# CityU-AIM-Group/SimT

Measured on AMD Instinct MI355X. Metric: training images/sec at 768x768, DeepLabv2-R101+SimT, higher is better.
Workload: dtype bf16

## Files before the change

simt_amd/csrc/bn_pool.hip:

```cpp
#include "common.h"

template <int NJ>
__device__ __forceinline__ void part_colsum8(const float* part, int nblk, int C, int c0, double* out , double (*red)[8][NJ]) {
  const int cl = threadIdx.x & 7, r = threadIdx.x >> 3;
  const int c = c0 + cl;
  double s[NJ];
#pragma unroll
  for (int j = 0; j < NJ; ++j) s[j] = 0.0;
  if (c < C) {
    int b = r;
    for (; b + 96 < nblk; b += 128) {
      float v[4][NJ];
#pragma unroll
      for (int u = 0; u < 4; ++u)
#pragma unroll
        for (int j = 0; j < NJ; ++j) v[u][j] = part[((long)(b + 32 * u) * NJ + j) * C + c];
#pragma unroll
      for (int u = 0; u < 4; ++u)
#pragma unroll
        for (int j = 0; j < NJ; ++j) s[j] += (double)v[u][j];
    }
    for (; b < nblk; b += 32)
#pragma unroll
      for (int j = 0; j < NJ; ++j) s[j] += (double)part[((long)b * NJ + j) * C + c];
// ... 35 lines not shown
    running_mean[c] = (1.f - momentum) * running_mean[c] + momentum * (float)mean;
    running_var[c] = (1.f - momentum) * running_var[c] + momentum * (float)unb;
  }
}

extern "C" int simt_bn_finalize(const float* part, int nblk, int C, long count, const float* gamma, const float* beta,
                                float* running_mean, float* running_var, float momentum, float eps, float* mean,
                                float* rstd, float* scale, float* shift, simt_stream_t stream) {
  SIMT_CHECK(part && mean && rstd && scale && shift && C > 0 && nblk > 0);
  hipLaunchKernelGGL(bn_finalize_kernel, dim3((C + 7) / 8), dim3(256), 0, (hipStream_t)stream, part, nblk, C, count,
                     gamma, beta, running_mean, running_var, momentum, eps, mean, rstd, scale, shift);
  SIMT_LAUNCH_CHECK();
  return SIMT_OK;
}

template <typename T>
__global__ void bn_apply_kernel(const T* y, const float* scale, const float* shift, const T* res, const T* y2,
                                const float* scale2, const float* shift2, T* z, unsigned char* bits, long nvec, int C, int relu) {
  const int vpr = C >> 3;
  const long i0 = (long)blockIdx.x * blockDim.x + threadIdx.x;
  const int c = (int)(i0 % vpr) << 3;
  float sc[8], sh[8], sc2[8], sh2[8];
  load8(scale + c, sc);
  load8(shift + c, sh);
  if (y2) { load8(scale2 + c, sc2); load8(shift2 + c, sh2); }
  for (long i = i0; i < nvec; i += (long)gridDim.x * blockDim.x) {
    float v[8];
    load8(y + i * 8, v);
#pragma unroll
    for (int e = 0; e < 8; ++e) v[e] = v[e] * sc[e] + sh[e];
    if (res) {
      float r[8];
      load8(res + i * 8, r);
#pragma unroll
      for (int e = 0; e < 8; ++e) v[e] += r[e];
    }
    if (y2) {
      float r[8];
      load8(y2 + i * 8, r);
#pragma unroll
      for (int e = 0; e < 8; ++e) v[e] += r[e] * sc2[e] + sh2[e];
    }
    if (relu) {
#pragma unroll
      for (int e = 0; e < 8; ++e) v[e] = v[e] > 0.f ? v[e] : 0.f;
    }
    store8(z + i * 8, v);
    if (bits) {
      unsigned b = 0;
#pragma unroll
      for (int e = 0; e < 8; ++e) b |= (v[e] > 0.f ? 1u : 0u) << e;
      bits[i] = (unsigned char)b;
    }
  }
}

static inline int ew_grid(long nvec) {
  long g = (nvec + 255) / 256;
  if (g > 256 * 16) g = 256 * 16;
  if (g < 1) g = 1;
  return (int)g;
}

extern "C" int simt_bn_apply_bits(const void* y, const float* scale, const float* shift, const void* res, const void* y2,
                                  const float* scale2, const float* shift2, void* z, unsigned char* bits, long M, int C,
                                  int relu, int dtype, simt_stream_t stream) {
  SIMT_CHECK(y && scale && shift && z && C % 8 == 0 && 256 % (C / 8) == 0);
  long nvec = M * (C / 8);
  if (dtype == SIMT_BF16)
    hipLaunchKernelGGL(bn_apply_kernel<bf16_t>, dim3(ew_grid(nvec)), dim3(256), 0, (hipStream_t)stream, (const bf16_t*)y,
                       scale, shift, (const bf16_t*)res, (const bf16_t*)y2, scale2, shift2, (bf16_t*)z, bits, nvec, C, relu);
  else
    hipLaunchKernelGGL(bn_apply_kernel<float>, dim3(ew_grid(nvec)), dim3(256), 0, (hipStream_t)stream, (const float*)y,
                       scale, shift, (const float*)res, (const float*)y2, scale2, shift2, (float*)z, bits, nvec, C, relu);
  SIMT_LAUNCH_CHECK();
  return SIMT_OK;
}
extern "C" int simt_bn_apply(const void* y, const float* scale, const float* shift, const void* res, const void* y2,
                             const float* scale2, const float* shift2, void* z, long M, int C, int relu, int dtype,
                             simt_stream_t stream) {
  return simt_bn_apply_bits(y, scale, shift, res, y2, scale2, shift2, z, nullptr, M, C, relu, dtype, stream);
}

template <typename T>
__global__ __launch_bounds__(256) void bn_bwd_reduce_kernel(const T* dz, const T* z, const T* y, const float* mean,
                                                           const float* rstd, const float* scale, const float* shift,
                                                           const T* y2, const float* mean2, const float* rstd2,
                                                           float* part, long M, int C, int rows_per_block,
                                                           int mask_mode) {
  __shared__ float red[3][256][8 + 1];
  const int vpr = C >> 3;
  const int rpar = 256 / vpr;
  const int tid = threadIdx.x;
  const int vc = tid % vpr, rl = tid / vpr;
  const int c = vc << 3;
  float mu[8], rs[8], sc[8], sh[8], mu2[8], rs2[8];
  load8(mean + c, mu);
  load8(rstd + c, rs);
  if (mask_mode == 2) { load8(scale + c, sc); load8(shift + c, sh); }
  if (y2) { load8(mean2 + c, mu2); load8(rstd2 + c, rs2); }
  float s1[8], s2[8], s3[8];
#pragma unroll
  for (int e = 0; e < 8; ++e) { s1[e] = 0.f; s2[e] = 0.f; s3[e] = 0.f; }
  long r0 = (long)blockIdx.x * rows_per_block;
  long r1 = r0 + rows_per_block;
  if (r1 > M) r1 = M;
  auto row = [&](const Raw8<T>& gq, const Raw8<T>& yq, const Raw8<T>& zq, unsigned b, const Raw8<T>& y2q) {
    float g[8], yv[8];
    raw8_unpack(gq, g);
    raw8_unpack(yq, yv);
    if (mask_mode == 1) {
      float zv[8];
      raw8_unpack(zq, zv);
#pragma unroll
      for (int e = 0; e < 8; ++e) g[e] = zv[e] > 0.f ? g[e] : 0.f;
    } else if (mask_mode == 2) {
#pragma unroll
      for (int e = 0; e < 8; ++e) g[e] = (yv[e] * sc[e] + sh[e]) > 0.f ? g[e] : 0.f;
    } else if (mask_mode == 3) {
#pragma unroll
      for (int e = 0; e < 8; ++e) g[e] = ((b >> e) & 1u) ? g[e] : 0.f;
    }
#pragma unroll
    for (int e = 0; e < 8; ++e) {
      s1[e] += g[e];
      s2[e] += g[e] * ((yv[e] - mu[e]) * rs[e]);
    }
    if (y2) {
      float y2v[8];
      raw8_unpack(y2q, y2v);
#pragma unroll
      for (int e = 0; e < 8; ++e) s3[e] += g[e] * ((y2v[e] - mu2[e]) * rs2[e]);
    }
  };
  if (rl < rpar) {
    constexpr int UR = 4;
    long r = r0 + rl;
    for (; r + (long)(UR - 1) * rpar < r1; r += (long)UR * rpar) {
      Raw8<T> gq[UR], yq[UR], zq[UR], y2q[UR];
      unsigned b[UR];
#pragma unroll
      for (int u = 0; u < UR; ++u) {
        const long off = (r + (long)u * rpar) * C + c;
        raw8_load(dz + off, gq[u]);
        raw8_load(y + off, yq[u]);
        if (mask_mode == 1) raw8_load(z + off, zq[u]); else zq[u] = gq[u];
        b[u] = mask_mode == 3 ? ((const unsigned char*)z)[off >> 3] : 0u;
        if (y2) raw8_load(y2 + off, y2q[u]); else y2q[u] = gq[u];
      }
#pragma unroll
      for (int u = 0; u < UR; ++u) row(gq[u], yq[u], zq[u], b[u], y2q[u]);
    }
    for (; r < r1; r += rpar) {
      const long off = r * C + c;
      Raw8<T> gq, yq, zq, y2q;
      raw8_load(dz + off, gq);
      raw8_load(y + off, yq);
      if (mask_mode == 1) raw8_load(z + off, zq); else zq = gq;
      const unsigned b = mask_mode == 3 ? ((const unsigned char*)z)[off >> 3] : 0u;
      if (y2) raw8_load(y2 + off, y2q); else y2q = gq;
      row(gq, yq, zq, b, y2q);
    }
  }
#pragma unroll
  for (int e = 0; e < 8; ++e) { red[0][tid][e] = s1[e]; red[1][tid][e] = s2[e]; red[2][tid][e] = s3[e]; }
  __syncthreads();
  for (int idx = tid; idx < 3 * C; idx += 256) {
    int j = idx / C, cc = idx - j * C;
    int v = cc >> 3, e = cc & 7;
    float s = 0.f;
    for (int q = 0; q < rpar; ++q) s += red[j][q * vpr + v][e];
    part[((long)blockIdx.x * 3 + j) * C + cc] = s;
  }
}

__global__ __launch_bounds__(256, 8) void bn_bwd_finalize_kernel(const float* part, int nblk, int C, long count, float* coef,
                                                             float* dgamma, float* dbeta, float* dgamma2, float* dbeta2) {
  __shared__ double red[32][8][3];
  double s[3];
  part_colsum8<3>(part, nblk, C, blockIdx.x * 8, s, red);
  const int c = blockIdx.x * 8 + (threadIdx.x & 7);
  if ((threadIdx.x >> 3) != 0 || c >= C) return;
#pragma unroll
  for (int j = 0; j < 3; ++j) coef[j * C + c] = (float)(s[j] / (double)count);
  if (dbeta) dbeta[c] = (float)s[0];
  if (dgamma) dgamma[c] = (float)s[1];
  if (dbeta2) dbeta2[c] = (float)s[0];
  if (dgamma2) dgamma2[c] = (float)s[2];
}

template <typename T>
__global__ void bn_bwd_apply_kernel(const T* dz, const T* z, const T* y, const float* mean, const float* rstd,
                                    const float* scale, const float* shift, const float* coef, const T* y2,
                                    const float* mean2, const float* rstd2, const float* scale2, T* dy, T* dy2, T* gout,
                                    long nvec, int C, int mask_mode) {
  const int vpr = C >> 3;
  const long i0 = (long)blockIdx.x * blockDim.x + threadIdx.x;
  const int c = (int)(i0 % vpr) << 3;
  float mu[8], rs[8], sc[8], c1[8], c2[8], sh[8], mu2[8], rs2[8], sc2[8], c3[8];
  load8(mean + c, mu);
  load8(rstd + c, rs);
  load8(scale + c, sc);
  load8(coef + c, c1);
  load8(coef + C + c, c2);
  if (mask_mode == 2) load8(shift + c, sh);
  if (y2) { load8(mean2 + c, mu2); load8(rstd2 + c, rs2); load8(scale2 + c, sc2); load8(coef + 2 * C + c, c3); }
  for (long i = i0; i < nvec; i += (long)gridDim.x * blockDim.x) {
    float g[8], yv[8];
    load8(dz + i * 8, g);
    load8(y + i * 8, yv);
    if (mask_mode == 1) {
      float zv[8];
      load8(z + i * 8, zv);
#pragma unroll
      for (int e = 0; e < 8; ++e) g[e] = zv[e] > 0.f ? g[e] : 0.f;
    } else if (mask_mode == 2) {
#pragma unroll
      for (int e = 0; e < 8; ++e) g[e] = (yv[e] * sc[e] + sh[e]) > 0.f ? g[e] : 0.f;
    } else if (mask_mode == 3) {
      const unsigned b = ((const unsigned char*)z)[i];
#pragma unroll
      for (int e = 0; e < 8; ++e) g[e] = ((b >> e) & 1u) ? g[e] : 0.f;
    }
    float o[8];
#pragma unroll
    for (int e = 0; e < 8; ++e) o[e] = sc[e] * (g[e] - c1[e] - ((yv[e] - mu[e]) * rs[e]) * c2[e]);
    store8(dy + i * 8, o);
    if (y2) {
      float y2v[8];
      load8(y2 + i * 8, y2v);
#pragma unroll
      for (int e = 0; e < 8; ++e) o[e] = sc2[e] * (g[e] - c1[e] - ((y2v[e] - mu2[e]) * rs2[e]) * c3[e]);
      store8(dy2 + i * 8, o);
    }
    if (gout) store8(gout + i * 8, g);
  }
}

#ifndef SIMT_BNB_APPLY4
#define SIMT_BNB_APPLY4 1
#endif
__device__ __forceinline__ void load4(const float* p, float* v) { const float4 a = *(const float4*)p; v[0] = a.x; v[1] = a.y; v[2] = a.z; v[3] = a.w; }
__device__ __forceinline__ void unpack4(const uint2& r, float* v) {
  v[0] = __uint_as_float(r.x << 16); v[1] = __uint_as_float(r.x & 0xffff0000u);
  v[2] = __uint_as_float(r.y << 16); v[3] = __uint_as_float(r.y & 0xffff0000u);
}
#ifndef SIMT_BNB_APPLY4_UN
#define SIMT_BNB_APPLY4_UN 1
#endif
template <int MM>
__global__ __launch_bounds__(256, 8) void bn_bwd_apply4_kernel(const bf16_t* dz, const bf16_t* z, const bf16_t* y, const float* mean, const float* rstd,
                                                               const float* scale, const float* shift, const float* coef, bf16_t* dy, bf16_t* gout,
                                                               long nvec4, int C) {
  constexpr int UN = SIMT_BNB_APPLY4_UN;
  const int vpr = C >> 2;
  const long i0 = (long)blockIdx.x * blockDim.x + threadIdx.x;
  const int c = (int)(i0 % vpr) << 2;
  float mu[4], rs[4], sc[4], c1[4], c2[4], sh[4];
  load4(mean + c, mu);
  load4(rstd + c, rs);
  load4(scale + c, sc);
  load4(coef + c, c1);
  load4(coef + C + c, c2);
  if (MM == 2) load4(shift + c, sh);
  const unsigned nb = (unsigned)nvec4 * 8u, Sb = gridDim.x * blockDim.x * 8u;
  const char* dzb = (const char*)dz; const char* yb = (const char*)y; const char* zb = (const char*)z;
  char* dyb = (char*)dy; char* gb = (char*)gout;
  for (unsigned o0 = (unsigned)i0 * 8u; o0 < nb; o0 += Sb * UN) {
    uint2 gr[UN], yr[UN], zr[UN];
    unsigned bb[UN];
#pragma unroll
    for (int u = 0; u < UN; ++u) {
      const unsigned ou = o0 + u * Sb < nb ? o0 + u * Sb : o0;
      gr[u] = *(const uint2*)(dzb + ou);
      yr[u] = *(const uint2*)(yb + ou);
      if (MM == 1) zr[u] = *(const uint2*)(zb + ou);
      if (MM == 3) bb[u] = (unsigned)((const unsigned char*)zb)[ou >> 4] >> ((ou >> 1) & 4u);
    }
#pragma unroll
    for (int u = 0; u < UN; ++u) {
      const unsigned ou = o0 + u * Sb;
      if (ou >= nb) break;
      float g[4], yv[4];
      unpack4(gr[u], g);
      unpack4(yr[u], yv);
      if (MM == 1) {
        float zv[4];
        unpack4(zr[u], zv);
#pragma unroll
        for (int e = 0; e < 4; ++e) g[e] = zv[e] > 0.f ? g[e] : 0.f;
      } else if (MM == 2) {
#pragma unroll
        for (int e = 0; e < 4; ++e) g[e] = (yv[e] * sc[e] + sh[e]) > 0.f ? g[e] : 0.f;
      } else if (MM == 3) {
#pragma unroll
        for (int e = 0; e < 4; ++e) g[e] = ((bb[u] >> e) & 1u) ? g[e] : 0.f;
      }
      float o[4];
#pragma unroll
      for (int e = 0; e < 4; ++e) o[e] = sc[e] * (g[e] - c1[e] - ((yv[e] - mu[e]) * rs[e]) * c2[e]);
      *(uint2*)(dyb + ou) = make_uint2(pack_bf16x2(o[0], o[1]), pack_bf16x2(o[2], o[3]));
      if (gout) *(uint2*)(gb + ou) = make_uint2(pack_bf16x2(g[0], g[1]), pack_bf16x2(g[2], g[3]));
    }
  }
}

static inline int bn_bwd_rows_per_block(long M, int C) {
  int rpar = 256 / (C / 8);
  long target_blocks = 512;
  long rpb = (M + target_blocks - 1) / target_blocks;
  rpb = ((rpb + rpar - 1) / rpar) * rpar;
  if (rpb < rpar * 4) rpb = rpar * 4;
  return (int)rpb;
}

extern "C" int simt_bn_bwd_nblk(long M, int C) {
  int rpb = bn_bwd_rows_per_block(M, C);
  return (int)((M + rpb - 1) / rpb);
}

extern "C" int simt_bn_bwd(const simt_bn_bwd_desc* d, simt_stream_t stream) {
  SIMT_CHECK(d && d->dz && d->y && d->mean && d->rstd && d->scale && d->part && d->coef && d->dy);
  SIMT_CHECK(d->C % 8 == 0 && d->C / 8 <= 256 && 256 % (d->C / 8) == 0);
  SIMT_CHECK((d->mask_mode != 1 && d->mask_mode != 3) || d->z);
  SIMT_CHECK(d->mask_mode != 2 || d->shift);
  SIMT_CHECK(!d->y2 || (d->mean2 && d->rstd2 && d->scale2 && d->dy2));
  hipStream_t st = (hipStream_t)stream;
  const int rpb = bn_bwd_rows_per_block(d->M, d->C);
  const int nblk = d->reduce_done_nblk > 0 ? d->reduce_done_nblk : (int)((d->M + rpb - 1) / rpb);
  const long nvec = d->M * (d->C / 8);
  if (d->reduce_done_nblk > 0) {
    SIMT_CHECK(!d->y2);
  } else if (d->dtype == SIMT_BF16) {
    hipLaunchKernelGGL(bn_bwd_reduce_kernel<bf16_t>, dim3(nblk), dim3(256), 0, st, (const bf16_t*)d->dz,
                       (const bf16_t*)d->z, (const bf16_t*)d->y, d->mean, d->rstd, d->scale, d->shift,
                       (const bf16_t*)d->y2, d->mean2, d->rstd2, d->part, d->M, d->C, rpb, d->mask_mode);
  } else {
    hipLaunchKernelGGL(bn_bwd_reduce_kernel<float>, dim3(nblk), dim3(256), 0, st, (const float*)d->dz,
                       (const float*)d->z, (const float*)d->y, d->mean, d->rstd, d->scale, d->shift,
                       (const float*)d->y2, d->mean2, d->rstd2, d->part, d->M, d->C, rpb, d->mask_mode);
  }
  SIMT_LAUNCH_CHECK();
  hipLaunchKernelGGL(bn_bwd_finalize_kernel, dim3((d->C + 7) / 8), dim3(256), 0, st, d->part, nblk, d->C, d->M, d->coef,
                     d->dgamma, d->dbeta, d->dgamma2, d->dbeta2);
  SIMT_LAUNCH_CHECK();
  if (SIMT_BNB_APPLY4 && d->dtype == SIMT_BF16 && !d->y2 && nvec * 16 < (1l << 31)) {
#ifndef SIMT_BNB_APPLY4_CAP
#define SIMT_BNB_APPLY4_CAP 4096
#endif
    long gl = (nvec * 2 + 256l * SIMT_BNB_APPLY4_UN - 1) / (256l * SIMT_BNB_APPLY4_UN);
    int g4 = (int)(gl > SIMT_BNB_APPLY4_CAP ? SIMT_BNB_APPLY4_CAP : gl < 1 ? 1 : gl);
    if (d->C / 4 > 256) g4 = (g4 + 1) & ~1;
#define SIMT_BNB4(MM) hipLaunchKernelGGL(bn_bwd_apply4_kernel<MM>, dim3(g4), dim3(256), 0, st, (const bf16_t*)d->dz, (const bf16_t*)d->z, (const bf16_t*)d->y, \
                                         d->mean, d->rstd, d->scale, d->shift, d->coef, (bf16_t*)d->dy, (bf16_t*)d->gout, nvec * 2, d->C)
    if (d->mask_mode == 3) SIMT_BNB4(3); else if (d->mask_mode == 2) SIMT_BNB4(2); else if (d->mask_mode == 1) SIMT_BNB4(1); else SIMT_BNB4(0);
#undef SIMT_BNB4
  } else if (d->dtype == SIMT_BF16) {
    hipLaunchKernelGGL(bn_bwd_apply_kernel<bf16_t>, dim3(ew_grid(nvec)), dim3(256), 0, st, (const bf16_t*)d->dz,
                       (const bf16_t*)d->z, (const bf16_t*)d->y, d->mean, d->rstd, d->scale, d->shift, d->coef,
                       (const bf16_t*)d->y2, d->mean2, d->rstd2, d->scale2, (bf16_t*)d->dy, (bf16_t*)d->dy2,
                       (bf16_t*)d->gout, nvec, d->C, d->mask_mode);
  } else {
    hipLaunchKernelGGL(bn_bwd_apply_kernel<float>, dim3(ew_grid(nvec)), dim3(256), 0, st, (const float*)d->dz,
                       (const float*)d->z, (const float*)d->y, d->mean, d->rstd, d->scale, d->shift, d->coef,
                       (const float*)d->y2, d->mean2, d->rstd2, d->scale2, (float*)d->dy, (float*)d->dy2,
                       (float*)d->gout, nvec, d->C, d->mask_mode);
  }
  SIMT_LAUNCH_CHECK();
  return SIMT_OK;
}

template <typename T, int KHC, int KWC>
__global__ void im2col_stem_kernel(const float* x, T* A, int B, int Cin, int H, int W, int Ho, int Wo, int KHr, int KWr,
                                   int stride, int pad, int ldk, long nvec) {
// ... 501 lines not shown
```

simt_amd/csrc/conv_wgrad2.hip:

```cpp
#include "common.h"
#include <stdlib.h>
#include <type_traits>

struct Wgrad2KArgs {
  const char* dy;
  const char* x;
  float* slab;
  const char* zero;
  int H, W, Cin, Ho, Wo, Cd, ldd, stride, ntaps, M, Ktot;
  int nsplit, pix_per_split, cotiles, ktiles;
  int tile0;
  float rcpWo, rcpHoWo;
  short tdy[SIMT_MAX_TAPS], tdx[SIMT_MAX_TAPS];
};

template <int N> __device__ __forceinline__ void wg_wait_vmcnt() {
  if constexpr (N == 0) asm volatile("s_waitcnt vmcnt(0)" ::: "memory");
  else asm volatile("s_waitcnt vmcnt(6)" ::: "memory");
}

template <int MODE>
__device__ __forceinline__ void conv_wgrad2_body(const Wgrad2KArgs& a, const int split, const int tix) {
  constexpr int NT = 512, NST = 3, BP = 64;
  constexpr int ROWB = 256;
// ... 109 lines not shown
    offa[t] = (8 * g + q) * ROWB + ((((cba >> 3) + (pp >> 1)) ^ hh) << 4) + (pp & 1) * 8;
    offb[t] = (1 + (wn >> 1)) * SUB + (8 * g + q) * ROWB + ((((cbb >> 3) + (pp >> 1)) ^ hh) << 4) + (pp & 1) * 8;
  }
  bf16x8 af[2][4], bfr[2][4];
  auto trd = [](unsigned addr, auto off) {
    bf16x4 r;
    asm volatile("ds_read_b64_tr_b16 %0, %1 offset:%2" : "=v"(r) : "v"(addr), "n"(decltype(off)::value));
    return r;
  };
  auto load_frags = [&](int buf) {
    const unsigned base = (unsigned)(size_t)LPTR(smem + buf * STAGE);
#pragma unroll
    for (int t = 0; t < 4; ++t) {
      const unsigned pa = base + (unsigned)offa[t], pb = base + (unsigned)offb[t];
      {
        const bf16x4 a0 = trd(pa, std::integral_constant<int, 0>{}), a1 = trd(pa, std::integral_constant<int, 4 * ROWB>{});
        const bf16x4 b0 = trd(pb, std::integral_constant<int, 0>{}), b1 = trd(pb, std::integral_constant<int, 4 * ROWB>{});
        af[0][t] = __builtin_shufflevector(a0, a1, 0, 1, 2, 3, 4, 5, 6, 7);
        bfr[0][t] = __builtin_shufflevector(b0, b1, 0, 1, 2, 3, 4, 5, 6, 7);
      }
      {
        const bf16x4 a0 = trd(pa, std::integral_constant<int, 32 * ROWB>{}), a1 = trd(pa, std::integral_constant<int, 36 * ROWB>{});
        const bf16x4 b0 = trd(pb, std::integral_constant<int, 32 * ROWB>{}), b1 = trd(pb, std::integral_constant<int, 36 * ROWB>{});
        af[1][t] = __builtin_shufflevector(a0, a1, 0, 1, 2, 3, 4, 5, 6, 7);
        bfr[1][t] = __builtin_shufflevector(b0, b1, 0, 1, 2, 3, 4, 5, 6, 7);
      }
    }
  };
  auto frags_landed = [&]() {
    asm volatile("s_waitcnt lgkmcnt(0)" : "+v"(af[0][0]), "+v"(af[0][1]), "+v"(af[0][2]), "+v"(af[0][3]), "+v"(af[1][0]), "+v"(af[1][1]), "+v"(af[1][2]), "+v"(af[1][3]));
    asm volatile("" : "+v"(bfr[0][0]), "+v"(bfr[0][1]), "+v"(bfr[0][2]), "+v"(bfr[0][3]), "+v"(bfr[1][0]), "+v"(bfr[1][1]), "+v"(bfr[1][2]), "+v"(bfr[1][3]));
  };
  auto mma = [&]() {
#pragma unroll
    for (int ks = 0; ks < 2; ++ks)
#pragma unroll
      for (int i = 0; i < 4; ++i)
#pragma unroll
        for (int j = 0; j < 4; ++j)
          acc[i][j] = __builtin_amdgcn_mfma_f32_16x16x32_bf16(bfr[ks][j], af[ks][i], acc[i][j], 0, 0, 0);
  };

  if (MODE != 2) {
    if (nk > 0) issue(0);
    if (nk > 1) issue(1);
  }
  int buf = 0;
  if (wave < 4) {
    for (int kt = 0; kt < nk; ++kt) {
      if (kt + 1 < nk) wg_wait_vmcnt<6>(); else wg_wait_vmcnt<0>();
      __builtin_amdgcn_s_barrier();
      asm volatile("" ::: "memory");
      if (MODE != 1) load_frags(buf);
      if (MODE != 2 && kt + 2 < nk) issue(buf >= 1 ? buf - 1 : NST - 1);
      if (MODE != 1) { frags_landed(); mma(); }
      buf = (buf + 1 == NST) ? 0 : buf + 1;
    }
  } else {
    for (int kt = 0; kt < nk; ++kt) {
      if (kt + 1 < nk) wg_wait_vmcnt<6>(); else wg_wait_vmcnt<0>();
      asm volatile("s_waitcnt lgkmcnt(0)" ::: "memory");
      __builtin_amdgcn_s_barrier();
      asm volatile("" ::: "memory");
      if (MODE != 1 && kt > 0) { frags_landed(); mma(); }
      if (MODE != 2 && kt + 2 < nk) issue(buf >= 1 ? buf - 1 : NST - 1);
      if (MODE != 1) load_frags(buf);
      buf = (buf + 1 == NST) ? 0 : buf + 1;
    }
    if (MODE != 1 && nk > 0) { frags_landed(); mma(); }
  }

  float* out = a.slab + (long)split * a.Cd * a.Ktot;
#pragma unroll
  for (int i = 0; i < 4; ++i)
#pragma unroll
    for (int j = 0; j < 4; ++j) {
      const int co = co0 + wm * 64 + i * 16 + (lane & 15);
      const int k = k0 + wn * 64 + j * 16 + (lane >> 4) * 4;
      if (co < a.Cd && k < a.Ktot) st_out16f(out + (long)co * a.Ktot + k, acc[i][j]);
    }
}


template <int MODE>
__device__ __forceinline__ void conv_wgrad3_body(const Wgrad2KArgs& a, const int split, const int tix) {
  constexpr int NST = 4, BP = 32;
  constexpr int ROWB = 256;
  constexpr int SUB = BP * ROWB;
  constexpr int STAGE = 4 * SUB;
  extern __shared__ __attribute__((aligned(16))) char smem[];

  const int tid = threadIdx.x;
  const int lane = tid & 63;
  const int wave = __builtin_amdgcn_readfirstlane(tid >> 6);
  const int wm = wave >> 2, wn = wave & 3;

  const int kt_ = tix % a.ktiles, ct = tix / a.ktiles;
  const int co0 = ct * 256, k0 = kt_ * 256;

  const int c_pos = tid & 15;
  const int row = tid >> 4;
  const int h = ((row & 3) | (((row >> 3) & 1) << 2)) << 1;
  const int cg = c_pos ^ h;
  int dch[2], xoff[2], tdy[2], tdx[2];
  bool d_ok[2], k_ok[2];
#pragma unroll
  for (int s = 0; s < 2; ++s) {
    dch[s] = co0 + s * 128 + cg * 8;
    d_ok[s] = dch[s] < a.Cd;
    const int kk = k0 + s * 128 + cg * 8;
    k_ok[s] = kk < a.Ktot;
    int tap = 0, ci = 0;
    if (k_ok[s]) { tap = kk / a.Cin; ci = kk - tap * a.Cin; }
    tdy[s] = a.tdy[tap];
    tdx[s] = a.tdx[tap];
    xoff[s] = ((tdy[s] * a.W + tdx[s]) * a.Cin + ci) * 2;
  }
  const int pix_bytes = a.Cin * 2;
  const int ldd_bytes = a.ldd * 2;
  const int HoWo = a.Ho * a.Wo;
  const bool s1 = a.stride == 1;

  const int m_begin = split * a.pix_per_split;
  int m_end = m_begin + a.pix_per_split;
  if (m_end > a.M) m_end = a.M;
  const int nk = (m_end > m_begin) ? (m_end - m_begin + BP - 1) / BP : 0;
  const char* zsrc = a.zero + c_pos * 16;

  int ld_m = m_begin;
  int r_oy, r_ox;
  unsigned r_xo, r_do;
  const int adv_r = BP % HoWo;
  const int adv_y = adv_r / a.Wo, adv_x = adv_r % a.Wo;
  {
    const int m = m_begin + row;
    int b, r;
    fast_divmod(m < a.M ? m : 0, HoWo, a.rcpHoWo, b, r);
    fast_divmod(r, a.Wo, a.rcpWo, r_oy, r_ox);
    r_xo = (unsigned)m * (unsigned)pix_bytes;
    r_do = (unsigned)m * (unsigned)ldd_bytes;
  }
  const unsigned x_step = (unsigned)BP * (unsigned)pix_bytes, d_step = (unsigned)BP * (unsigned)ldd_bytes;
  auto issue = [&](int buf) {
    char* sbase = smem + buf * STAGE + wave * 1024;
    const int m = ld_m + row;
    const bool mok = m < m_end;
    const char* srcd[2];
    const char* srcx[2];
    if (s1) {
#pragma unroll
      for (int s = 0; s < 2; ++s) {
        srcd[s] = (mok && d_ok[s]) ? a.dy + (r_do + (unsigned)(dch[s] * 2)) : zsrc;
        const bool in = (unsigned)(r_oy + tdy[s]) < (unsigned)a.H && (unsigned)(r_ox + tdx[s]) < (unsigned)a.W;
        srcx[s] = (mok && k_ok[s] && in) ? a.x + (r_xo + (unsigned)xoff[s]) : zsrc;
      }
      r_do += d_step; r_xo += x_step;
      r_oy += adv_y; r_ox += adv_x;
      if (r_ox >= a.Wo) { r_ox -= a.Wo; r_oy += 1; }
      if (r_oy >= a.Ho) r_oy -= a.Ho;
    } else {
      int b, r, oy, ox;
      fast_divmod(m, HoWo, a.rcpHoWo, b, r);
      fast_divmod(r, a.Wo, a.rcpWo, oy, ox);
#pragma unroll
      for (int s = 0; s < 2; ++s) {
        srcd[s] = (mok && d_ok[s]) ? a.dy + ((unsigned)m * (unsigned)ldd_bytes + (unsigned)(dch[s] * 2)) : zsrc;
        srcx[s] = zsrc;
        const int iy = oy * a.stride + tdy[s], ix = ox * a.stride + tdx[s];
        if (mok && k_ok[s] && iy >= 0 && iy < a.H && ix >= 0 && ix < a.W)
          srcx[s] = a.x + ((unsigned)((b * a.H + iy) * a.W + ix) * (unsigned)pix_bytes + (unsigned)(xoff[s] - (tdy[s] * a.W + tdx[s]) * pix_bytes));
      }
    }
    if (MODE != 2) {
      __builtin_amdgcn_global_load_lds(GPTR(srcd[0]), LPTR(sbase), 16, 0, 0);
      __builtin_amdgcn_global_load_lds(GPTR(srcd[1]), LPTR(sbase + SUB), 16, 0, 0);
      __builtin_amdgcn_global_load_lds(GPTR(srcx[0]), LPTR(sbase + 2 * SUB), 16, 0, 0);
      __builtin_amdgcn_global_load_lds(GPTR(srcx[1]), LPTR(sbase + 3 * SUB), 16, 0, 0);
    }
    ld_m += BP;
  };

  f32x4 acc[8][4];
#pragma unroll
  for (int i = 0; i < 8; ++i)
#pragma unroll
    for (int j = 0; j < 4; ++j) acc[i][j] = (f32x4){0.f, 0.f, 0.f, 0.f};

  const int g = lane >> 4, q = (lane & 15) >> 2, pp = lane & 3;
  const int hh = (q | ((g & 1) << 2)) << 1;
  const unsigned rowpart = (unsigned)((8 * g + q) * ROWB + (pp & 1) * 8);
  unsigned offa[8], offb[4];
#pragma unroll
  for (int t = 0; t < 8; ++t) offa[t] = (unsigned)(wm * SUB) + rowpart + (unsigned)((((t * 2) + (pp >> 1)) ^ hh) << 4);
#pragma unroll
  for (int t = 0; t < 4; ++t) offb[t] = (unsigned)((2 + (wn >> 1)) * SUB) + rowpart + (unsigned)((((((wn & 1) * 64 + t * 16) >> 3) + (pp >> 1)) ^ hh) << 4);
  bf16x8 af[8], bfr[4];
  auto trd = [](unsigned addr, auto off) {
    bf16x4 r;
    asm volatile("ds_read_b64_tr_b16 %0, %1 offset:%2" : "=v"(r) : "v"(addr), "n"(decltype(off)::value));
    return r;
  };
  auto load_frags = [&](int buf) {
    const unsigned base = (unsigned)(size_t)LPTR(smem + buf * STAGE);
#pragma unroll
    for (int t = 0; t < 4; ++t) {
      const bf16x4 b0 = trd(base + offb[t], std::integral_constant<int, 0>{}), b1 = trd(base + offb[t], std::integral_constant<int, 4 * ROWB>{});
      bfr[t] = __builtin_shufflevector(b0, b1, 0, 1, 2, 3, 4, 5, 6, 7);
    }
#pragma unroll
    for (int t = 0; t < 8; ++t) {
      const bf16x4 a0 = trd(base + offa[t], std::integral_constant<int, 0>{}), a1 = trd(base + offa[t], std::integral_constant<int, 4 * ROWB>{});
      af[t] = __builtin_shufflevector(a0, a1, 0, 1, 2, 3, 4, 5, 6, 7);
    }
  };
  auto frags_landed = [&]() {
    asm volatile("s_waitcnt lgkmcnt(0)" : "+v"(af[0]), "+v"(af[1]), "+v"(af[2]), "+v"(af[3]), "+v"(af[4]), "+v"(af[5]), "+v"(af[6]), "+v"(af[7]));
    asm volatile("" : "+v"(bfr[0]), "+v"(bfr[1]), "+v"(bfr[2]), "+v"(bfr[3]));
  };
  auto mma = [&]() {
#pragma unroll
    for (int i = 0; i < 8; ++i)
#pragma unroll
      for (int j = 0; j < 4; ++j)
        acc[i][j] = __builtin_amdgcn_mfma_f32_16x16x32_bf16(bfr[j], af[i], acc[i][j], 0, 0, 0);
  };
  auto wait_stage = [&](int kt) {
    if (kt + 2 < nk) asm volatile("s_waitcnt vmcnt(8)" ::: "memory");
    else if (kt + 1 < nk) asm volatile("s_waitcnt vmcnt(4)" ::: "memory");
    else asm volatile("s_waitcnt vmcnt(0)" ::: "memory");
  };

#pragma unroll
  for (int s = 0; s < NST - 1; ++s) if (s < nk) issue(s);
  int buf = 0;
  if (wave < 4) {
    for (int kt = 0; kt < nk; ++kt) {
      wait_stage(kt);
      __builtin_amdgcn_s_barrier();
      asm volatile("" ::: "memory");
      if (MODE != 1) load_frags(buf);
      if (kt + NST - 1 < nk) issue(buf >= 1 ? buf - 1 : NST - 1);
      if (MODE != 1) { frags_landed(); mma(); }
      buf = (buf + 1 == NST) ? 0 : buf + 1;
    }
  } else {
    for (int kt = 0; kt < nk; ++kt) {
      wait_stage(kt);
      asm volatile("s_waitcnt lgkmcnt(0)" ::: "memory");
      __builtin_amdgcn_s_barrier();
      asm volatile("" ::: "memory");
      if (MODE != 1 && kt > 0) { frags_landed(); mma(); }
      if (kt + NST - 1 < nk) issue(buf >= 1 ? buf - 1 : NST - 1);
      if (MODE != 1) load_frags(buf);
      buf = (buf + 1 == NST) ? 0 : buf + 1;
    }
    if (MODE != 1 && nk > 0) { frags_landed(); mma(); }
  }

  float* out = a.slab + (long)split * a.Cd * a.Ktot;
#pragma unroll
  for (int i = 0; i < 8; ++i)
#pragma unroll
    for (int j = 0; j < 4; ++j) {
      const int co = co0 + wm * 128 + i * 16 + (lane & 15);
      const int k = k0 + wn * 64 + j * 16 + (lane >> 4) * 4;
      if (co < a.Cd && k < a.Ktot) st_out16f(out + (long)co * a.Ktot + k, acc[i][j]);
    }
}

template <int MODE>
__global__ __launch_bounds__(512, 2) void conv_wgrad2_kernel(Wgrad2KArgs a) {
  const int tiles = a.cotiles * a.ktiles;
  const int lin = xcd_remap(blockIdx.x, tiles * a.nsplit);
  const int split = lin / tiles;
  conv_wgrad2_body<MODE>(a, split, lin - split * tiles);
}

__global__ __launch_bounds__(512, 2) void conv_wgrad2_multi_kernel(const Wgrad2KArgs* __restrict__ jobs, int njobs, int tiles) {
  const int lin = xcd_remap(blockIdx.x, (int)gridDim.x);
  const int split = lin / tiles;
  const int t = lin - split * tiles;
  int j = 0;
  for (int i = 1; i < njobs; ++i) if (t >= jobs[i].tile0) j = i;
  conv_wgrad2_body<0>(jobs[j], split, t - jobs[j].tile0);
}

template <int MODE>
__global__ __launch_bounds__(512, 2) void conv_wgrad3_kernel(Wgrad2KArgs a) {
  const int tiles = a.cotiles * a.ktiles;
  const int lin = xcd_remap(blockIdx.x, tiles * a.nsplit);
  const int split = lin / tiles;
  conv_wgrad3_body<MODE>(a, split, lin - split * tiles);
}
__global__ __launch_bounds__(512, 2) void conv_wgrad3_multi_kernel(const Wgrad2KArgs* __restrict__ jobs, int njobs, int tiles) {
// ... 127 lines not shown
```

Measured before the change: 173.5.

## Narrow BN-backward reduce to 4 channels per thread and slim wgrad3 address registers

The BN backward reduce kernel now has each thread handle 4 bf16 channels instead of 8, looping over 512 virtual threads per block. It specializes the kernel at compile time on mask mode and y2 presence, uses 32-bit offsets, and raises the occupancy hint. The apply4 kernel loads the shift vector inside the mask branch instead of keeping it in registers. The wgrad3 conv kernel replaces per-fragment LDS offset arrays with one base address XORed per tile, folds the k_ok check into an out-of-range tdy sentinel, and uses a single zero source, all to cut VGPR pressure. The changes risk more loop overhead and depend on the XOR addressing matching the original swizzle.

```diff
diff --git a/simt_amd/csrc/bn_pool.hip b/simt_amd/csrc/bn_pool.hip
--- a/simt_amd/csrc/bn_pool.hip
+++ b/simt_amd/csrc/bn_pool.hip
@@ -141,96 +141,143 @@
   return simt_bn_apply_bits(y, scale, shift, res, y2, scale2, shift2, z, nullptr, M, C, relu, dtype, stream);
 }
 
-template <typename T>
-__global__ __launch_bounds__(256) void bn_bwd_reduce_kernel(const T* dz, const T* z, const T* y, const float* mean,
+#ifndef SIMT_BNB_REDUCE4
+#define SIMT_BNB_REDUCE4 1
+#endif
+template <typename T> constexpr int bnb_reduce_cpt() { return (SIMT_BNB_REDUCE4 && std::is_same<T, bf16_t>::value) ? 4 : 8; }
+template <typename T> constexpr int bnb_reduce_threads() { return 2048 / bnb_reduce_cpt<T>(); }
+template <typename T> constexpr int bnb_reduce_pitch() { return bnb_reduce_cpt<T>() == 4 ? 4 : 9; }
+struct Raw4b { uint2 r; };
+__device__ __forceinline__ void bnb_load(const float* p, Raw8<float>& q) { raw8_load(p, q); }
+__device__ __forceinline__ void bnb_load(const bf16_t* p, Raw8<bf16_t>& q) { raw8_load(p, q); }
+__device__ __forceinline__ void bnb_load(const bf16_t* p, Raw4b& q) { q.r = *(const uint2*)p; }
+template <typename R> __device__ __forceinline__ void bnb_unpack(const R& q, float* v) { raw8_unpack(q, v); }
+__device__ __forceinline__ void bnb_unpack(const Raw4b& q, float* v) {
+  v[0] = __uint_as_float(q.r.x << 16); v[1] = __uint_as_float(q.r.x & 0xffff0000u);
+  v[2] = __uint_as_float(q.r.y << 16); v[3] = __uint_as_float(q.r.y & 0xffff0000u);
+}
+template <int N> __device__ __forceinline__ void bnb_loadc(const float* p, float* v) {
+  if constexpr (N == 4) { const float4 a = *(const float4*)p; v[0] = a.x; v[1] = a.y; v[2] = a.z; v[3] = a.w; }
+  else load8(p, v);
+}
+
+template <typename T, int MM, int Y2>
+__device__ __forceinline__ void bn_bwd_reduce_body(const T* dz, const T* z, const T* y, const float* mean, const float* rstd, const float* scale,
+                                                   const float* shift, const T* y2, const float* mean2, const float* rstd2, float* part, long M,
+                                                   int C, int rows_per_block, int mask_mode_rt,
+                                                   float (*red)[bnb_reduce_threads<T>()][bnb_reduce_pitch<T>()]) {
+  constexpr int CPT = bnb_reduce_cpt<T>();
+  constexpr int NT = bnb_reduce_threads<T>();
+  using Raw = std::conditional_t<CPT == 4, Raw4b, Raw8<T>>;
+  const int mask_mode = MM >= 0 ? MM : mask_mode_rt;
+  if (Y2 == 0) y2 = nullptr;
+  const int vpr = C / CPT;
+  const int rpar = NT / vpr;
+#pragma unroll 1
+  for (int vt = threadIdx.x; vt < NT; vt += 256) {
+  const int vc = vt % vpr, rl = vt / vpr;
+  const int c = vc * CPT;
+  float mu[CPT], rs[CPT], sc[CPT], sh[CPT], mu2[CPT], rs2[CPT];
+  bnb_loadc<CPT>(mean + c, mu);
+  bnb_loadc<CPT>(rstd + c, rs);
+  if (mask_mode == 2) { bnb_loadc<CPT>(scale + c, sc); bnb_loadc<CPT>(shift + c, sh); }
+  if (y2) { bnb_loadc<CPT>(mean2 + c, mu2); bnb_loadc<CPT>(rstd2 + c, rs2); }
+  float s1[CPT], s2[CPT], s3[CPT];
+#pragma unroll
+  for (int e = 0; e < CPT; ++e) { s1[e] = 0.f; s2[e] = 0.f; s3[e] = 0.f; }
+  long r0 = (long)blockIdx.x * rows_per_block;
+  long r1 = r0 + rows_per_block;
+  if (r1 > M) r1 = M;
+  auto row = [&](const Raw& gq, const Raw& yq, const Raw& zq, unsigned b, const Raw& y2q) {
+    float g[CPT], yv[CPT];
+    bnb_unpack(gq, g);
+    bnb_unpack(yq, yv);
+    if (mask_mode == 1) {
+      float zv[CPT];
+      bnb_unpack(zq, zv);
+#pragma unroll
+      for (int e = 0; e < CPT; ++e) g[e] = zv[e] > 0.f ? g[e] : 0.f;
+    } else if (mask_mode == 2) {
+#pragma unroll
+      for (int e = 0; e < CPT; ++e) g[e] = (yv[e] * sc[e] + sh[e]) > 0.f ? g[e] : 0.f;
+    } else if (mask_mode == 3) {
+#pragma unroll
+      for (int e = 0; e < CPT; ++e) g[e] = ((b >> e) & 1u) ? g[e] : 0.f;
+    }
+#pragma unroll
+    for (int e = 0; e < CPT; ++e) {
+      s1[e] += g[e];
+      s2[e] += g[e] * ((yv[e] - mu[e]) * rs[e]);
+    }
+    if (y2) {
+      float y2v[CPT];
+      bnb_unpack(y2q, y2v);
+#pragma unroll
+      for (int e = 0; e < CPT; ++e) s3[e] += g[e] * ((y2v[e] - mu2[e]) * rs2[e]);
+    }
+  };
+  const unsigned bsh = (unsigned)(c & 7);
+  if (rl < rpar) {
+    const long e0 = r0 * C;
+    const T* dzr = dz + e0; const T* yr = y + e0; const T* zr = mask_mode == 1 ? z + e0 : z; const T* y2r = y2 ? y2 + e0 : y2;
+    const unsigned char* br = (const unsigned char*)z + (e0 >> 3);
+    const unsigned ostep = (unsigned)rpar * (unsigned)C;
+    constexpr int UR = 4;
+    long r = r0 + rl;
+    unsigned o = (unsigned)rl * (unsigned)C + (unsigned)c;
+    for (; r + (long)(UR - 1) * rpar < r1; r += (long)UR * rpar, o += UR * ostep) {
+      Raw gq[UR], yq[UR], zq[UR], y2q[UR];
+      unsigned b[UR];
+#pragma unroll
+      for (int u = 0; u < UR; ++u) {
+        const unsigned off = o + u * ostep;
+        bnb_load(dzr + off, gq[u]);
+        bnb_load(yr + off, yq[u]);
+        if (mask_mode == 1) bnb_load(zr + off, zq[u]); else zq[u] = gq[u];
+        b[u] = mask_mode == 3 ? (unsigned)br[off >> 3] >> bsh : 0u;
+        if (y2) bnb_load(y2r + off, y2q[u]); else y2q[u] = gq[u];
+      }
+#pragma unroll
+      for (int u = 0; u < UR; ++u) row(gq[u], yq[u], zq[u], b[u], y2q[u]);
+    }
+    for (; r < r1; r += rpar, o += ostep) {
+      Raw gq, yq, zq, y2q;
+      bnb_load(dzr + o, gq);
+      bnb_load(yr + o, yq);
+      if (mask_mode == 1) bnb_load(zr + o, zq); else zq = gq;
+      const unsigned b = mask_mode == 3 ? (unsigned)br[o >> 3] >> bsh : 0u;
+      if (y2) bnb_load(y2r + o, y2q); else y2q = gq;
+      row(gq, yq, zq, b, y2q);
+    }
+  }
+#pragma unroll
+  for (int e = 0; e < CPT; ++e) { red[0][vt][e] = s1[e]; red[1][vt][e] = s2[e]; red[2][vt][e] = s3[e]; }
+  }
+  __syncthreads();
+  for (int idx = threadIdx.x; idx < 3 * C; idx += 256) {
+    int j = idx / C, cc = idx - j * C;
+    int v = cc / CPT, e = cc % CPT;
+    float s = 0.f;
+    for (int q = 0; q < rpar; ++q) s += red[j][q * vpr + v][e];
+    part[((long)blockIdx.x * 3 + j) * C + cc] = s;
+  }
+}
+
+template <typename T>
+__global__ __launch_bounds__(256, bnb_reduce_cpt<T>() == 4 ? 6 : 1) void bn_bwd_reduce_kernel(const T* dz, const T* z, const T* y, const float* mean,
                                                            const float* rstd, const float* scale, const float* shift,
                                                            const T* y2, const float* mean2, const float* rstd2,
                                                            float* part, long M, int C, int rows_per_block,
                                                            int mask_mode) {
-  __shared__ float red[3][256][8 + 1];
-  const int vpr = C >> 3;
-  const int rpar = 256 / vpr;
-  const int tid = threadIdx.x;
-  const int vc = tid % vpr, rl = tid / vpr;
-  const int c = vc << 3;
-  float mu[8], rs[8], sc[8], sh[8], mu2[8], rs2[8];
-  load8(mean + c, mu);
-  load8(rstd + c, rs);
-  if (mask_mode == 2) { load8(scale + c, sc); load8(shift + c, sh); }
-  if (y2) { load8(mean2 + c, mu2); load8(rstd2 + c, rs2); }
-  float s1[8], s2[8], s3[8];
-#pragma unroll
-  for (int e = 0; e < 8; ++e) { s1[e] = 0.f; s2[e] = 0.f; s3[e] = 0.f; }
-  long r0 = (long)blockIdx.x * rows_per_block;
-  long r1 = r0 + rows_per_block;
-  if (r1 > M) r1 = M;
-  auto row = [&](const Raw8<T>& gq, const Raw8<T>& yq, const Raw8<T>& zq, unsigned b, const Raw8<T>& y2q) {
-    float g[8], yv[8];
-    raw8_unpack(gq, g);
-    raw8_unpack(yq, yv);
-    if (mask_mode == 1) {
-      float zv[8];
-      raw8_unpack(zq, zv);
-#pragma unroll
-      for (int e = 0; e < 8; ++e) g[e] = zv[e] > 0.f ? g[e] : 0.f;
-    } else if (mask_mode == 2) {
-#pragma unroll
-      for (int e = 0; e < 8; ++e) g[e] = (yv[e] * sc[e] + sh[e]) > 0.f ? g[e] : 0.f;
-    } else if (mask_mode == 3) {
-#pragma unroll
-      for (int e = 0; e < 8; ++e) g[e] = ((b >> e) & 1u) ? g[e] : 0.f;
-    }
-#pragma unroll
-    for (int e = 0; e < 8; ++e) {
-      s1[e] += g[e];
-      s2[e] += g[e] * ((yv[e] - mu[e]) * rs[e]);
-    }
-    if (y2) {
-      float y2v[8];
-      raw8_unpack(y2q, y2v);
-#pragma unroll
-      for (int e = 0; e < 8; ++e) s3[e] += g[e] * ((y2v[e] - mu2[e]) * rs2[e]);
-    }
-  };
-  if (rl < rpar) {
-    constexpr int UR = 4;
-    long r = r0 + rl;
-    for (; r + (long)(UR - 1) * rpar < r1; r += (long)UR * rpar) {
-      Raw8<T> gq[UR], yq[UR], zq[UR], y2q[UR];
-      unsigned b[UR];
-#pragma unroll
-      for (int u = 0; u < UR; ++u) {
-        const long off = (r + (long)u * rpar) * C + c;
-        raw8_load(dz + off, gq[u]);
-        raw8_load(y + off, yq[u]);
-        if (mask_mode == 1) raw8_load(z + off, zq[u]); else zq[u] = gq[u];
-        b[u] = mask_mode == 3 ? ((const unsigned char*)z)[off >> 3] : 0u;
-        if (y2) raw8_load(y2 + off, y2q[u]); else y2q[u] = gq[u];
-      }
-#pragma unroll
-      for (int u = 0; u < UR; ++u) row(gq[u], yq[u], zq[u], b[u], y2q[u]);
-    }
-    for (; r < r1; r += rpar) {
-      const long off = r * C + c;
-      Raw8<T> gq, yq, zq, y2q;
-      raw8_load(dz + off, gq);
-      raw8_load(y + off, yq);
-      if (mask_mode == 1) raw8_load(z + off, zq); else zq = gq;
-      const unsigned b = mask_mode == 3 ? ((const unsigned char*)z)[off >> 3] : 0u;
-      if (y2) raw8_load(y2 + off, y2q); else y2q = gq;
-      row(gq, yq, zq, b, y2q);
-    }
-  }
-#pragma unroll
-  for (int e = 0; e < 8; ++e) { red[0][tid][e] = s1[e]; red[1][tid][e] = s2[e]; red[2][tid][e] = s3[e]; }
-  __syncthreads();
-  for (int idx = tid; idx < 3 * C; idx += 256) {
-    int j = idx / C, cc = idx - j * C;
-    int v = cc >> 3, e = cc & 7;
-    float s = 0.f;
-    for (int q = 0; q < rpar; ++q) s += red[j][q * vpr + v][e];
-    part[((long)blockIdx.x * 3 + j) * C + cc] = s;
-  }
+  __shared__ float red[3][bnb_reduce_threads<T>()][bnb_reduce_pitch<T>()];
+#define SIMT_BNBR(MM, Y2) bn_bwd_reduce_body<T, MM, Y2>(dz, z, y, mean, rstd, scale, shift, y2, mean2, rstd2, part, M, C, rows_per_block, mask_mode, red)
+  if constexpr (bnb_reduce_cpt<T>() == 4) {
+    if (y2) { if (mask_mode == 3) SIMT_BNBR(3, 1); else if (mask_mode == 2) SIMT_BNBR(2, 1); else if (mask_mode == 1) SIMT_BNBR(1, 1); else SIMT_BNBR(0, 1); }
+    else { if (mask_mode == 3) SIMT_BNBR(3, 0); else if (mask_mode == 2) SIMT_BNBR(2, 0); else if (mask_mode == 1) SIMT_BNBR(1, 0); else SIMT_BNBR(0, 0); }
+  } else {
+    SIMT_BNBR(-1, -1);
+  }
+#undef SIMT_BNBR
 }
 
 __global__ __launch_bounds__(256, 8) void bn_bwd_finalize_kernel(const float* part, int nblk, int C, long count, float* coef,
@@ -307,6 +354,9 @@
 #ifndef SIMT_BNB_APPLY4_UN
 #define SIMT_BNB_APPLY4_UN 1
 #endif
+#ifndef SIMT_BNB_APPLY4_RELOAD
+#define SIMT_BNB_APPLY4_RELOAD 1
+#endif
 template <int MM>
 __global__ __launch_bounds__(256, 8) void bn_bwd_apply4_kernel(const bf16_t* dz, const bf16_t* z, const bf16_t* y, const float* mean, const float* rstd,
                                                                const float* scale, const float* shift, const float* coef, bf16_t* dy, bf16_t* gout,
@@ -321,7 +371,7 @@
   load4(scale + c, sc);
   load4(coef + c, c1);
   load4(coef + C + c, c2);
-  if (MM == 2) load4(shift + c, sh);
+  if (MM == 2 && !SIMT_BNB_APPLY4_RELOAD) load4(shift + c, sh);
   const unsigned nb = (unsigned)nvec4 * 8u, Sb = gridDim.x * blockDim.x * 8u;
   const char* dzb = (const char*)dz; const char* yb = (const char*)y; const char* zb = (const char*)z;
   char* dyb = (char*)dy; char* gb = (char*)gout;
@@ -349,6 +399,7 @@
 #pragma unroll
         for (int e = 0; e < 4; ++e) g[e] = zv[e] > 0.f ? g[e] : 0.f;
       } else if (MM == 2) {
+        if (SIMT_BNB_APPLY4_RELOAD) load4(shift + c, sh);
 #pragma unroll
         for (int e = 0; e < 4; ++e) g[e] = (yv[e] * sc[e] + sh[e]) > 0.f ? g[e] : 0.f;
       } else if (MM == 3) {
diff --git a/simt_amd/csrc/conv_wgrad2.hip b/simt_amd/csrc/conv_wgrad2.hip
--- a/simt_amd/csrc/conv_wgrad2.hip
+++ b/simt_amd/csrc/conv_wgrad2.hip
@@ -215,6 +215,9 @@
 }
 
 
+#ifndef SIMT_WGRAD3_LEAN
+#define SIMT_WGRAD3_LEAN 1
+#endif
 template <int MODE>
 __device__ __forceinline__ void conv_wgrad3_body(const Wgrad2KArgs& a, const int split, const int tix) {
   constexpr int NST = 4, BP = 32;
@@ -248,6 +251,9 @@
     tdy[s] = a.tdy[tap];
     tdx[s] = a.tdx[tap];
     xoff[s] = ((tdy[s] * a.W + tdx[s]) * a.Cin + ci) * 2;
+#if SIMT_WGRAD3_LEAN
+    if (!k_ok[s]) tdy[s] = 1 << 20;
+#endif
   }
   const int pix_bytes = a.Cin * 2;
   const int ldd_bytes = a.ldd * 2;
@@ -258,7 +264,11 @@
   int m_end = m_begin + a.pix_per_split;
   if (m_end > a.M) m_end = a.M;
   const int nk = (m_end > m_begin) ? (m_end - m_begin + BP - 1) / BP : 0;
+#if SIMT_WGRAD3_LEAN
+  const char* zsrc = a.zero;
+#else
   const char* zsrc = a.zero + c_pos * 16;
+#endif
 
   int ld_m = m_begin;
   int r_oy, r_ox;
@@ -272,6 +282,9 @@
     fast_divmod(r, a.Wo, a.rcpWo, r_oy, r_ox);
     r_xo = (unsigned)m * (unsigned)pix_bytes;
     r_do = (unsigned)m * (unsigned)ldd_bytes;
+#if SIMT_WGRAD3_LEAN
+    r_do += (unsigned)(dch[0] * 2);
+#endif
   }
   const unsigned x_step = (unsigned)BP * (unsigned)pix_bytes, d_step = (unsigned)BP * (unsigned)ldd_bytes;
   auto issue = [&](int buf) {
@@ -283,9 +296,15 @@
     if (s1) {
 #pragma unroll
       for (int s = 0; s < 2; ++s) {
+#if SIMT_WGRAD3_LEAN
+        srcd[s] = (mok && d_ok[s]) ? a.dy + (r_do + (unsigned)(s * 256)) : zsrc;
+        const bool in = (unsigned)(r_oy + tdy[s]) < (unsigned)a.H && (unsigned)(r_ox + tdx[s]) < (unsigned)a.W;
+        srcx[s] = (mok && in) ? a.x + (r_xo + (unsigned)xoff[s]) : zsrc;
+#else
         srcd[s] = (mok && d_ok[s]) ? a.dy + (r_do + (unsigned)(dch[s] * 2)) : zsrc;
         const bool in = (unsigned)(r_oy + tdy[s]) < (unsigned)a.H && (unsigned)(r_ox + tdx[s]) < (unsigned)a.W;
         srcx[s] = (mok && k_ok[s] && in) ? a.x + (r_xo + (unsigned)xoff[s]) : zsrc;
+#endif
       }
       r_do += d_step; r_xo += x_step;
       r_oy += adv_y; r_ox += adv_x;
@@ -322,11 +341,16 @@
   const int g = lane >> 4, q = (lane & 15) >> 2, pp = lane & 3;
   const int hh = (q | ((g & 1) << 2)) << 1;
   const unsigned rowpart = (unsigned)((8 * g + q) * ROWB + (pp & 1) * 8);
+#if SIMT_WGRAD3_LEAN
+  const unsigned la = (unsigned)(wm * SUB) + rowpart + (unsigned)((((pp >> 1)) | hh) << 4);
+  const unsigned lb = (unsigned)((2 + (wn >> 1)) * SUB) + rowpart + (unsigned)(((((wn & 1) * 8) + (pp >> 1)) ^ hh) << 4);
+#else
   unsigned offa[8], offb[4];
 #pragma unroll
   for (int t = 0; t < 8; ++t) offa[t] = (unsigned)(wm * SUB) + rowpart + (unsigned)((((t * 2) + (pp >> 1)) ^ hh) << 4);
 #pragma unroll
   for (int t = 0; t < 4; ++t) offb[t] = (unsigned)((2 + (wn >> 1)) * SUB) + rowpart + (unsigned)((((((wn & 1) * 64 + t * 16) >> 3) + (pp >> 1)) ^ hh) << 4);
+#endif
   bf16x8 af[8], bfr[4];
   auto trd = [](unsigned addr, auto off) {
     bf16x4 r;
@@ -335,14 +359,27 @@
   };
   auto load_frags = [&](int buf) {
     const unsigned base = (unsigned)(size_t)LPTR(smem + buf * STAGE);
+#if SIMT_WGRAD3_LEAN
+    const unsigned pa = base + la, pb = base + lb;
+#endif
 #pragma unroll
     for (int t = 0; t < 4; ++t) {
-      const bf16x4 b0 = trd(base + offb[t], std::integral_constant<int, 0>{}), b1 = trd(base + offb[t], std::integral_constant<int, 4 * ROWB>{});
+#if SIMT_WGRAD3_LEAN
+      const unsigned ab = pb ^ (unsigned)(t << 5);
+#else
+      const unsigned ab = base + offb[t];
+#endif
+      const bf16x4 b0 = trd(ab, std::integral_constant<int, 0>{}), b1 = trd(ab, std::integral_constant<int, 4 * ROWB>{});
       bfr[t] = __builtin_shufflevector(b0, b1, 0, 1, 2, 3, 4, 5, 6, 7);
     }
 #pragma unroll
     for (int t = 0; t < 8; ++t) {
-      const bf16x4 a0 = trd(base + offa[t], std::integral_constant<int, 0>{}), a1 = trd(base + offa[t], std::integral_constant<int, 4 * ROWB>{});
+#if SIMT_WGRAD3_LEAN
+      const unsigned aa = pa ^ (unsigned)(t << 5);
+#else
+      const unsigned aa = base + offa[t];
+#endif
+      const bf16x4 a0 = trd(aa, std::integral_constant<int, 0>{}), a1 = trd(aa, std::integral_constant<int, 4 * ROWB>{});
       af[t] = __builtin_shufflevector(a0, a1, 0, 1, 2, 3, 4, 5, 6, 7);
     }
   };
```

New measurement: 174.3 (median of 6 runs). Within noise of the previous version (+0.5%).
